# HDembinski/zenflow

Hardware: AMD Instinct MI355X
Metric: log_prob samples/sec (+ NLL match) 4D 16-knot 4-layer flow, batch 2^20 (higher is better)
Workload: dtype fp32 (f16x2 split MFMA, fp32 accumulate)

## Files before the change

### zenflow_amd/csrc/zf_flow.hip

```cpp
#include "zf_flow_dev.h"

#include <cmath>
#include <cstdlib>
#include <cstring>
#include <vector>

namespace zf {
namespace {

constexpr int kWaves = 4;
constexpr int kBlockRows = kWaves * kTile;

template <int T>
__device__ __forceinline__ floatx16 mfma_tile(const floatx4* __restrict__ p,
                                              const floatx4* __restrict__ pnext, floatx4 (&cur)[4],
                                              const floatx16 (&hb)[T]) {
  floatx16 acc = floatx16{0};
#pragma unroll
  for (int t = 0; t < T; ++t) {
    floatx4 nxt[4];
    const bool more = (t + 1 < T);
    const floatx4* src = more ? p + (t + 1) * 256 : pnext;
    const bool have = more || (pnext != nullptr);
    if (have) {
// ... 192 lines not shown

  flow_epilogue<kWaves>(F, xs, s, hh, lane, wave, rot, D, row, valid, ld, lp_out, block_partial, 1, 0,
                        y_out, ld_out, s_part);
}

__global__ __launch_bounds__(256) void latent_sample_kernel(int latent, float param, unsigned long long seed,
                                                            float* __restrict__ z, long long n, int D) {
  const long long i = (long long)blockIdx.x * 256 + threadIdx.x;
  if (i >= n) return;
  const long long row = i / D;
  const int d = (int)(i - row * D);
  z[i] = latent_draw(latent, param, seed, row, d);
}

constexpr int kReduceThreads = 1024;
__global__ __launch_bounds__(kReduceThreads) void reduce_partials(const double* __restrict__ part, long long n,
                                                                  double* __restrict__ out) {
  __shared__ double sm[kReduceThreads];
  const int t = threadIdx.x;
  double acc = 0.0;
  long long i = t;
  for (; i + 7 * kReduceThreads < n; i += 8 * kReduceThreads) {
    double v[8];
#pragma unroll
    for (int j = 0; j < 8; ++j) v[j] = part[i + j * kReduceThreads];
#pragma unroll
    for (int j = 0; j < 8; ++j) acc += v[j];
  }
  for (; i < n; i += kReduceThreads) acc += part[i];
  sm[t] = acc;
// ... 349 lines not shown
  if (e == hipSuccess && layered) {
    rcd = zf::layered_create(desc, nat, need, &h->lay);
    if (rcd) {
      zf_flow_destroy(h);
      return rcd;
    }
  }
  if (e == hipSuccess && use_x3) e = hipMalloc(&h->d_x3, x3s.size() * sizeof(uint16_t));
  if (e == hipSuccess && use_x3)
    e = hipMemcpy(h->d_x3, x3s.data(), x3s.size() * sizeof(uint16_t), hipMemcpyHostToDevice);
  if (e == hipSuccess) e = hipMalloc(&h->d_desc, sizeof(zf::DevFlow));
  if (e == hipSuccess) e = hipMalloc(&h->d_blob, h->packed.size() * sizeof(float) + 1024);
  if (e == hipSuccess) e = hipMemcpy(h->d_desc, &h->host, sizeof(zf::DevFlow), hipMemcpyHostToDevice);
  if (e == hipSuccess)
    e = hipMemcpy(h->d_blob, h->packed.data(), h->packed.size() * sizeof(float), hipMemcpyHostToDevice);
  if (e != hipSuccess) {
    rcd = zf::hip_status(e, "zf_flow_create");
    zf_flow_destroy(h);
    return rcd;
  }
  *handle = h;
  return ZF_OK;
}

int zf_flow_destroy(zf_flow_t* h) {
  if (!h) return ZF_OK;
  if (h->d_desc) (void)hipFree(h->d_desc);
  if (h->d_blob) (void)hipFree(h->d_blob);
  if (h->d_x3) (void)hipFree(h->d_x3);
  if (h->d_res_state) (void)hipFree(h->d_res_state);
// ... 43 lines not shown
    a.oact = h->x3_oact;
    a.aset = h->x3_aset;
    a.par_bytes = h->host.x3_par_bytes;
    a.seed = seed;
    a.gen = gen;
    a.stream = (hipStream_t)stream;
    a.latent = h->host.latent;
    a.sb_affine = true;
    for (int i = op_begin; i < op_end; ++i) {
      if (h->desc.ops[i].kind != ZF_OP_SHIFT_BOUNDS) continue;
      for (int j = 0; j < h->host.D; ++j) {
        const int mode = (int)h->packed[(size_t)h->host.ops[i].sb + 8 * j];
        if (mode != ZF_SB_NONE && mode != ZF_SB_BOTH) a.sb_affine = false;
      }
    }
    if (h->x3_res_mode != 0 && (h->x3_res_mode == 1 || N >= kX3ResidentAutoRows) &&
        x3_resident_fits(h->desc, a, INV, h->ncu)) {
      const long long need = ((long long)(N + kTile - 1) / kTile) * kTile * (h->host.D + 1);
      if (need > h->res_floats) {
        hipStreamCaptureStatus cs = hipStreamCaptureStatusNone;
        if (hipStreamIsCapturing(a.stream, &cs) == hipSuccess && cs == hipStreamCaptureStatusNone) {
          if (h->d_res_state) (void)hipFree(h->d_res_state);
          h->d_res_state = nullptr;
          h->res_floats = 0;
          ZF_TRY_HIP(hipMalloc(&h->d_res_state, (size_t)need * sizeof(float)));
          h->res_floats = need;
        }
      }
      if (need <= h->res_floats) a.res_state = h->d_res_state;
    }
// ... 143 lines not shown
```

### zenflow_amd/csrc/zf_flow_dev.h

```cpp
#pragma once
#include "zf_act.h"
#include "zf_internal.h"
#include "zf_random.h"
#include "zf_spline.h"

#include <cstdint>
#include <vector>

namespace zf {

typedef float floatx16 __attribute__((ext_vector_type(16)));
typedef float floatx4 __attribute__((ext_vector_type(4)));

constexpr int kTile = 32;
constexpr int kMaxOps = 64;

struct DevOp {
  int kind, shift, K, S;
  int n_hidden, dt, dc, DC;
  int KS0, T_last, nslot_mask, act;
  long long w[17];
  long long b[17];
  long long bn;
  long long sb;
// ... 6 lines not shown
  float x3_rb[16][2];
  int x3_par_pieces;
  long long x3_nbase[2], x3_nbn[2];
  int x3_npieces[2], x3_npar[2];
};

struct DevFlow {
  int D, C, latent, n_ops;
  int HP, nslot, per_wave, x3_ok;
  int small_floats;
  int x3_par_bytes;
  int kreal;
  int _pad;
  float lat_c0, lat_c1, lat_c2, lat_c3;
  DevOp ops[kMaxOps];
};

__device__ __forceinline__ void wave_lds_sync() {
  __builtin_amdgcn_fence(__ATOMIC_SEQ_CST, "wavefront");
  __builtin_amdgcn_wave_barrier();
}

__device__ __forceinline__ float swish(float v) {
  return v * __builtin_amdgcn_rcpf(1.0f + __builtin_amdgcn_exp2f(-v * 1.44269504f));
}

__device__ __forceinline__ float rcp_refined(float x) {
  float r = __builtin_amdgcn_rcpf(x);
  return __builtin_fmaf(__builtin_fmaf(-x, r, 1.0f), r, r);
}
// ... 28 lines not shown
  floatx16 a;
#pragma unroll
  for (int r = 0; r < 16; ++r) a[r] = b[r >> 2][r & 3];
  return a;
}

__device__ __forceinline__ int pmod(int a, int m) {
  int r = a % m;
  return r < 0 ? r + m : r;
}

__device__ __forceinline__ int wrap(int a, int m) { return a >= m ? a - m : a; }

struct KnotConsts {
  float c, norm, rnorm;
  __device__ __forceinline__ explicit KnotConsts(int K) {
    const double c64 = 1e-5 / (1.0 - (double)K * 1e-5);
    c = (float)c64;
    norm = (float)(1.0 + c64 * (double)K);
    rnorm = rcp_refined(norm);
  }
};

__device__ __forceinline__ void load_state(float* xs, const float* __restrict__ xin, long long row,
                                           bool valid, int D, int s, int hh, const DevFlow* __restrict__ F,
                                           unsigned long long seed, int gen) {
  for (int d = hh; d < D; d += 2) {
    float v = 0.f;
    if (valid) v = gen ? latent_draw(F->latent, F->lat_c3, seed, row, d) : xin[row * D + d];
    xs[d * 32 + s] = v;
// ... 158 lines not shown
      if (lane == 0) s_part[wave] = v;
      __syncthreads();
      if (threadIdx.x == 0) {
        double acc = 0.0;
        for (int w = 0; w < NW; ++w) acc += s_part[w];
        const long long b0 = slot >= 0 ? slot : (long long)blockIdx.x * pstride;
        block_partial[b0] = acc;
        for (int k = 1; k < pstride; ++k)
          if (b0 + k < nparts) block_partial[b0 + k] = 0.0;
      }
    }
  }
  flow_out_rows(xs, s, hh, rot, D, row, valid, ld, y_out, ld_out);
}

struct X3Launch {
  const DevFlow* desc;
  const float* blob;
  const void* x3;
  const float *x, *c;
  float* y;
  const float* ld_in;
  float *ld_out, *lp;
  double* part;
  long long nparts;
  int op_begin, op_end;
  long long N;
  unsigned long long seed;
  int gen;
  int K, D, C, T;
  int NT;
  bool oact;
  int aset;
  int par_bytes;
  float* res_state = nullptr;
  int res_blocks = 0, res_slots = 0, res_span = 0;
  bool sb_affine = false;
  int latent = 0;
  bool res_frame = false;
  hipStream_t stream;
};
int launch_flow_x3(const X3Launch& a, bool inverse);
int x3_resident_mode();
bool x3_resident_fits(const zf_flow_desc& desc, X3Launch& a, bool inverse, int ncu);
bool x3_eligible(const zf_flow_desc& desc, int HP, int* K);
struct LayeredFlow;
int layered_create(const zf_flow_desc& desc, const float* natural, int64_t n, LayeredFlow** out);
void layered_destroy(LayeredFlow* L);
int layered_run(LayeredFlow* L, const DevFlow& F, const float* packed, bool inverse, int op_begin, int op_end,
                const float* x, const float* c, float* y, const float* ld_in, float* ld_out, float* lp, double* part,
                long long N, hipStream_t st, unsigned long long seed, int gen);
int x3_last_tiles(int K);
// ... 10 lines not shown
```

### zenflow_amd/csrc/zf_flow_x3.hip

```cpp
#include "zf_flow_x3_kernel.h"

#include <cmath>
#include <cstdint>
#include <cstdlib>
#include <cstring>
#include <vector>

namespace zf {

int launch_x3_k8(const X3Launch& a, bool inverse);
int launch_x3_k16(const X3Launch& a, bool inverse);
int launch_x3_k32(const X3Launch& a, bool inverse);
int launch_x3_k64(const X3Launch& a, bool inverse);

namespace {

uint16_t bf16_rne(float f) {
  uint32_t u;
  std::memcpy(&u, &f, 4);
  if ((u & 0x7fffffffu) > 0x7f800000u) return (uint16_t)((u >> 16) | 0x40);
  u += 0x7fffu + ((u >> 16) & 1u);
  return (uint16_t)(u >> 16);
}

// ... 47 lines not shown
    if (desc.ops[i].n_hidden != 2) return false;
    if (i >= a.op_begin && i < a.op_end) in_range = true;
  }
  if (!in_range) return false;
  const int TL = dt == 1 ? x3_last_tiles_one(a.K) : x3_last_tiles(a.K);
  const long long span = 4ll * (2 * 4 * 2 * 1024) + 4ll * (2 * TL * 2 * 1024);
  const long long nslots = (a.N + 127) / 128;
  const long long slots = (nslots + ncu - 1) / ncu;
  if (slots > (1 << 20)) return false;
  if (x3_res_lds_bytes((size_t)span, a.par_bytes, a.D + a.C, 4 * slots, false) > 160 * 1024) return false;
  if (a.K != 16 || dt != 2) return false;
#ifndef ZF_X3R_FRAME
#define ZF_X3R_FRAME 1
#endif
  a.res_frame = ZF_X3R_FRAME && a.D == 4 && a.C == 0 && a.sb_affine && a.latent == ZF_LATENT_NORMAL &&
                a.ld_in == nullptr;
  for (int i = a.op_begin, run = 0; i < a.op_end && a.res_frame; ++i) {
    const int kind = desc.ops[i].kind;
    run = kind == ZF_OP_NSC ? 0 : run + (kind == ZF_OP_SHIFT_BOUNDS ? 1 : 0);
    if (run > 1) a.res_frame = false;
  }
  if (x3_res_lds_bytes((size_t)span, a.par_bytes, a.D + a.C, 4 * slots, true) > 160 * 1024) a.res_frame = false;
  a.res_blocks = ncu;
  a.res_slots = (int)slots;
  a.res_span = (int)span;
  return true;
}

int x3_padded_knots(int K) {
  if (K < 2) return 0;
  if (K <= 8) return 8;
  if (K <= 16) return 16;
  if (K <= 32) return 32;
// ... 220 lines not shown
```

### zenflow_amd/csrc/zf_flow_x3_k16_res.hip

```cpp
#include "zf_flow_x3_kernel.h"

namespace zf {

int launch_x3r_k16(const X3Launch& a, bool inverse) { return launch_x3r<16, false>(a, inverse); }

}
```

### zenflow_amd/csrc/zf_flow_x3_kernel.h

```cpp
#pragma once
#include "zf_flow_dev.h"

#include <cmath>
#include <cstdint>
#include <cstdlib>
#include <cstring>
#include <utility>
#include <vector>

namespace zf {
namespace {

typedef float floatx2 __attribute__((ext_vector_type(2)));
typedef __bf16 bf16x2 __attribute__((ext_vector_type(2)));
typedef __bf16 bf16x8 __attribute__((ext_vector_type(8)));
typedef _Float16 halfx2 __attribute__((ext_vector_type(2)));
typedef _Float16 halfx8 __attribute__((ext_vector_type(8)));

template <int NT>
struct XT;
template <>
struct XT<3> {
  using E = bf16x8;
  static constexpr int kProd = 6;
// ... 7 lines not shown
constexpr int kWideSched = 3;

#ifndef ZF_X3_WAVES
#define ZF_X3_WAVES 4
#endif
constexpr int kX3Waves = ZF_X3_WAVES;
static_assert(kX3Waves % 4 == 0, "whole 128-row NLL partial slots per block");

#ifndef ZF_X3_ABL
#define ZF_X3_ABL 0
#endif
#ifdef ZF_X3_TRACE
constexpr int kX3TraceSlots = 16;
__device__ unsigned long long* x3_trace_buf;
#define X3T_NOW() __builtin_amdgcn_s_memtime()
#endif
template <int NT>
constexpr int group_bytes(int NOUT) { return 2 * NOUT * NT * 1024; }


template <int S>
__device__ __forceinline__ void split8(const floatx16& v, bf16x8& bh, bf16x8& bm, bf16x8& bl) {
#pragma unroll
  for (int i = 0; i < 4; ++i) {
    const floatx2 x = {v[8 * S + 2 * i], v[8 * S + 2 * i + 1]};
    const bf16x2 h = __builtin_convertvector(x, bf16x2);
    const floatx2 r = x - __builtin_convertvector(h, floatx2);
    const bf16x2 m = __builtin_convertvector(r, bf16x2);
    const floatx2 r2 = r - __builtin_convertvector(m, floatx2);
    const bf16x2 l = __builtin_convertvector(r2, bf16x2);
// ... 897 lines not shown
  }
}

template <int NT, int T, int NOUT, bool SW, bool OACT, int Q = 0>
__device__ __forceinline__ void x3_layer(const char* __restrict__ x3, X3Pipe& p, floatx16 (&hb)[T],
                                         floatx16 (&acc)[NOUT], int lane, const float* bias_last, int hh,
                                         float isc, float us, int act) {
  if constexpr (Q + 1 < T) {
    x3_step<NT, T, NOUT, Q, SW, OACT>(x3, p, hb, acc, lane, nullptr, hh, isc, us, act);
    x3_layer<NT, T, NOUT, SW, OACT, Q + 1>(x3, p, hb, acc, lane, bias_last, hh, isc, us, act);
  } else {
    x3_step<NT, T, NOUT, Q, SW, OACT>(x3, p, hb, acc, lane, bias_last, hh, isc, us, act);
  }
}

template <int T, bool OACT>
__device__ __forceinline__ void x3_layer0(const X3Sc& c, const float* par, const float* xs, int rot, int D,
                                          int s, int hh, int lane, floatx16 (&hb)[T], int swish_tiles,
                                          float* umax = nullptr) {
  const int dt = c.dt, dc = c.dc, DC = c.DC, KS0 = c.KS0;
  const int DCp = 2 * KS0;
  const float* bn = par;
  const float* w0b = par + c.w0_rel;
  const float* b0 = par + c.b_rel;
#pragma unroll
  for (int o = 0; o < T; ++o) hb[o] = bias_acc(b0 + o * 32, hh);
  for (int ks = 0; ks < KS0; ++ks) {
    const int k = 2 * ks + hh;
    float v = 0.f;
    if (k < dc) v = xs[wrap(dt + k + rot, D) * 32 + s];
    else if (k < DC) v = xs[(D + k - dc) * 32 + s];
    const float u = (v - bn[k]) * bn[DCp + k] + bn[2 * DCp + k];
    if (umax != nullptr) *umax = fmaxf(*umax, fabsf(u));
    const float* w0 = w0b + ks * 64 + lane;
#pragma unroll
    for (int o = 0; o < T; ++o) hb[o] = __builtin_amdgcn_mfma_f32_32x32x2f32(w0[o * KS0 * 64], u, hb[o], 0, 0, 0);
  }
#pragma unroll
  for (int o = 0; o < T; ++o)
    if (o < swish_tiles) {
      if constexpr (OACT) {
        x3_act_tile<3, true>(hb[o], 1.f, c.act);
      } else {
#pragma unroll
        for (int r = 0; r < 16; ++r) hb[o][r] = swish(hb[o][r]);
      }
    }
}

__device__ __forceinline__ float x3_squareplus(float x) {
  return 0.5f * (x + __builtin_amdgcn_sqrtf(__builtin_fmaf(x, x, 4.0f)));
}

__device__ __forceinline__ float x3_squareplus2(float x) {
  return x + __builtin_amdgcn_sqrtf(__builtin_fmaf(x, x, 4.0f));
}

__device__ __forceinline__ void x3_forward_eval(float x, const RqsBin& b, float& y, float& ld) {
  const float rw = rcp_refined(b.w);
  const float sk = b.h * rw;
  const float zr = (x - b.xk) * rw;
  const float z = (zr != zr) ? zr : fminf(fmaxf(zr, kEps), kOneMinusEps);
  const float az = 1.0f - z;
  const float num = b.h * z * (sk * z + b.dk * az);
  const float den = sk + (b.dkp1 + b.dk - 2.0f * sk) * z * az;
  const float rd = rcp_refined(den + kEps);
  const float yv = b.yk + num * rd;
  y = b.oob ? x : yv;
  const float num2 = z * (b.dkp1 * z + 2.0f * sk * az) + b.dk * (az * az);
  const float sq = (sk + kEps) * rd;
  const float l = __logf((num2 + kEps) * (sq * sq));
  ld = b.oob ? 0.0f : l;
}

__device__ __forceinline__ float x3_sqrt_cr(float a) {
  const float y = __builtin_amdgcn_rsqf(a);
  const float sq = a * y;
  const float r = __builtin_fmaf(__builtin_fmaf(-sq, sq, a), 0.5f * y, sq);
  return a == __builtin_huge_valf() ? a : r;
}
template <bool CR>
__device__ __forceinline__ float x3_squareplus2_t(float x) {
  const float a = __builtin_fmaf(x, x, 4.0f);
  return x + (CR ? x3_sqrt_cr(a) : __builtin_amdgcn_sqrtf(a));
}
// ... 24 lines not shown
    for (int i = 0; i <= H; ++i) S2[i] = c ? S[H + i] : S[i];
    x3_bsel<FWD, H, H>(v, X2, Y2, W2, H2, S2, out);
  }
}

template <int K>
struct KnotLit {
  static constexpr double c64 = 1e-5 / (1.0 - (double)K * 1e-5);
  static constexpr float c = (float)c64;
  static constexpr float norm = (float)(1.0 + c64 * (double)K);
  static constexpr float rnorm = (float)(1.0 / (double)norm);
  static constexpr float bc = c * rnorm;
};

template <bool FWD, int K, bool CR, bool KLIT, int NPV>
__device__ __forceinline__ RqsBin x3_bin(float v, const float (&P)[NPV], const KnotConsts& kc) {
  float ws[K], hs[K];
#pragma unroll
  for (int j = 0; j < K; ++j) {
    ws[j] = x3_squareplus2_t<CR>(P[j]);
    hs[j] = x3_squareplus2_t<CR>(P[K + j]);
  }
  float X[K + 1], Y[K + 1];
  X[0] = 0.f;
  Y[0] = 0.f;
  X[1] = ws[0];
  Y[1] = hs[0];
#pragma unroll
  for (int j = 1; j < K; ++j) {
    X[j + 1] = X[j] + ws[j];
    Y[j + 1] = Y[j] + hs[j];
  }
  const float rn = KLIT ? KnotLit<K>::rnorm : kc.rnorm;
  const float bc = KLIT ? KnotLit<K>::bc : kc.c * kc.rnorm;
  const float ax = rcp_refined(X[K]) * rn, ay = rcp_refined(Y[K]) * rn;
#pragma unroll
  for (int j = 1; j <= K; ++j) {
    const float jb = KLIT ? (float)j * KnotLit<K>::bc : (float)j * bc;
    X[j] = __builtin_fmaf(X[j], ax, jb);
    Y[j] = __builtin_fmaf(Y[j], ay, jb);
  }
  float S[K + 1];
  S[0] = 0.f;
  S[K] = 0.f;
#pragma unroll
  for (int j = 1; j < K; ++j) S[j] = P[2 * K + j - 1];
  float o[6];
  x3_bsel<FWD, K, K + 1>(v, X, Y, ws, hs, S, o);
  RqsBin b;
// ... 20 lines not shown
  unsigned long long t_last;
};
#define X3T(k)                                   \
  {                                              \
    const unsigned long long t_ = X3T_NOW();     \
    tr.tacc[k] += t_ - tr.t_last;                \
    tr.t_last = t_;                              \
  }
#elif defined(ZF_X3_MARK)
struct X3Tr {};
#define X3T(k) asm volatile(";ZFMARK " #k)
#else
struct X3Tr {};
#define X3T(k)
#endif
#ifdef ZF_X3_MARK
#define X3M(k) asm volatile(";ZFMARK " #k)
#else
#define X3M(k)
#endif

template <int NT, int K, int T, bool PAIRS, bool ONE, bool INV, bool OACT, int ASET, bool RES>
__device__ __forceinline__ void x3_nsc(const DevOp& op, const X3Sc& opc, const char* __restrict__ x3, X3Pipe& pipe,
                                       const float* par, float* xs, int rot, int D, int s, int hh, int lane,
                                       float& ld, X3Tr& tr) {
  constexpr int TL = ONE ? (3 * K - 1 + 31) / 32 : (3 * K - 1 + 15) / 16;
  constexpr int NPV = ONE ? 32 * TL : 16 * TL;
  const int nh = opc.nh, act = opc.act, dt = opc.dt, kw_last = opc.kw_last;
  const KnotConsts kc(opc.kreal);
  const bool padlast = opc.kreal == K - 1;
#ifdef ZF_X3_MARK
  const bool klit = true;
#else
  const bool klit = opc.kreal == K;
#endif
  const long long b_rel = opc.b_rel + T * 32, blast_rel = opc.blast_rel;
  floatx16 hb[T];
  constexpr bool kLastSW = !PAIRS;
  constexpr bool kPipe = T == 4 && !PAIRS;
#ifndef ZF_X3_EARLY
#define ZF_X3_EARLY 1
#endif
  constexpr bool kEarly = ZF_X3_EARLY && NT == 2 && !OACT && kPipe;
  static_assert(!RES || kEarly, "the resident form runs the early-scale slot schedule only");
#ifndef ZF_X3_PRESP
#define ZF_X3_PRESP 1
#endif
  constexpr int kPreSP = (!ZF_X3_PRESP || !kEarly) ? 0 : !ONE ? K / 8 : (K == 16 ? 1 : 0);
  float umax = 0.f;
  x3_layer0<T, OACT>(opc, par, xs, rot, D, s, hh, lane, hb, NT == 2 ? 0 : (!OACT && (nh > 1 || kLastSW)) ? 1 : T,
                     kEarly ? &umax : nullptr);
  float eU = 0.f, eisc = 1.f, eus = 1.f, eius = 1.f;
  halfx8 ecs[2];
  if constexpr (kEarly) {
    const X3Halves uq = x3_halves(umax);
    umax = fmaxf(uq.lo, uq.hi);
    eU = __builtin_fmaf(op.x3_rb[0][0], umax, op.x3_rb[0][1]);
    x3_scale_from(eU, nh > 1 ? opc.kw1 : kw_last, eisc, eus, eius);
    x3_act_tile<NT, false>(hb[0], eisc, act);
    split8h<0>(hb[0], ecs[0], ecs[1]);
  }
#ifndef ZF_X3_SEEDSCALED
#define ZF_X3_SEEDSCALED 0
#endif
  constexpr bool kSeedScaled = NT == 2 && (ZF_X3_SEEDSCALED || !kPipe);
#ifndef ZF_X3_WIDE_PIPE
#define ZF_X3_WIDE_PIPE 1
#endif
#ifndef ZF_X3_PAIRS_PIPE
#define ZF_X3_PAIRS_PIPE 1
#endif
  constexpr bool kPipeH = kPipe || (ZF_X3_PAIRS_PIPE && (T == 4 || ZF_X3_WIDE_PIPE) && NT == 2 && !OACT);
#ifndef ZF_X3_ACTIN
#define ZF_X3_ACTIN 1
#endif
  constexpr bool kActIn = ZF_X3_ACTIN && NT == 2 && ASET == 2 && kPipeH;
  constexpr bool kSeedScaledH = NT == 2 && (ZF_X3_SEEDSCALED || !kPipeH);
#if ZF_X3_ABL != 4
  if constexpr (T == 4) __builtin_amdgcn_s_setprio(2);
#endif
  X3T(1);
  if constexpr (kEarly) {
    float eM = eU;
    for (int l = 1; l < nh; ++l) {
      const float nU = __builtin_fmaf(op.x3_rb[l][0], eM, op.x3_rb[l][1]);
      float nisc, nus, nius;
      x3_scale_from(nU, l + 1 < nh ? op.x3_kw[l + 1] : kw_last, nisc, nus, nius);
      floatx16 acc[T];
#pragma unroll
      for (int o = 0; o < T; ++o) acc[o] = floatx16{0};
      float mx;
      x3_layer_early<T, T, true, 0, 0, RES>(x3, pipe, hb, acc, lane, par + b_rel + (l - 1) * (T * 32), hh, ecs, eisc, eus,
                                 nisc, mx);
#pragma unroll
      for (int o = 0; o < T; ++o) hb[o] = acc[o];
      eU = nU; eisc = nisc; eus = nus; eius = nius;
      const X3Halves mq = x3_halves(mx);
      eM = fmaxf(mq.lo, mq.hi);
    }
  } else
  for (int l = 1; l < nh; ++l) {
    floatx16 acc[T];
    float isc = 1.f, us = 1.f, ius = 1.f;
    if constexpr (NT == 2) {
      x3_act_scale<T, OACT>(hb, l == 1 ? opc.kw1 : op.x3_kw[l], isc, us, ius, act);
#pragma unroll
      for (int o = 0; o < (OACT && !kActIn ? T : 1); ++o) x3_act_tile<NT, OACT, ASET>(hb[o], isc, act);
    }
    const float* bl_l = par + b_rel + (l - 1) * (T * 32);
#pragma unroll
    for (int o = 0; o < T; ++o)
      acc[o] = NT == 3 ? bias_acc(bl_l + o * 32, hh)
                       : (kSeedScaledH ? bias_acc(bl_l + o * 32, hh) * ius : floatx16{0});
    const float* bh = (NT == 2 && !kSeedScaledH) ? bl_l : nullptr;
    if constexpr (kPipeH) {
      typename XT<NT>::E cs[NT];
      splitk<NT, 0>(hb[0], cs);
      halfx8 fs1[2];
      x3_layer_pipe<NT, T, T, NT == 2 && !kSeedScaledH, OACT, 0, kActIn ? ASET : 0>(x3, pipe, hb, acc, lane, bh, hh,
                                                                                 cs, isc, us,
// ... 9 lines not shown
#pragma unroll
    for (int o = 0; o < T; ++o) {
      if (o < nsw) {
        if constexpr (OACT) {
          hb[o] = acc[o];
          x3_act_tile<3, true>(hb[o], 1.f, act);
        } else {
#pragma unroll
          for (int r = 0; r < 16; ++r) hb[o][r] = swish(acc[o][r]);
        }
      } else {
        hb[o] = acc[o];
      }
    }
  }
  X3T(2);
  float ldn = 0.f;
  const int npair = PAIRS ? (dt + 1) / 2 : 1;
  float lisc = 1.f, lus = 1.f, lius = 1.f;
  if constexpr (kEarly) {
    lisc = eisc; lus = eus; lius = eius;
  } else if constexpr (NT == 2) {
    x3_act_scale<T, OACT>(hb, kw_last, lisc, lus, lius, act);
#pragma unroll
    for (int o = 0; o < T; ++o)
      if (o == 0 || !kLastSW || (OACT && !(kActIn && kPipe))) x3_act_tile<NT, OACT, ASET>(hb[o], lisc, act);
  }
#ifndef ZF_X3_PRESPLIT
#define ZF_X3_PRESPLIT 1
#endif
  constexpr bool kPre = ZF_X3_PRESPLIT && PAIRS && T == 4 && NT == 2 && !OACT;
  halfx8 sp[kPre ? T : 1][2][2];
  if constexpr (kPre) {
#pragma unroll
    for (int q = 0; q < T; ++q) {
      split8h<0>(hb[q], sp[q][0][0], sp[q][0][1]);
      split8h<1>(hb[q], sp[q][1][0], sp[q][1][1]);
    }
  }
  for (int pr = 0; pr < npair; ++pr) {
    const float* bl = par + blast_rel + pr * TL * 32;
    floatx16 pa[TL];
    constexpr bool kSeed = PAIRS && NT == 3;
#pragma unroll
    for (int o = 0; o < TL; ++o)
      pa[o] = kSeed ? bias_acc(bl + o * 32, hh) : (kSeedScaled ? bias_acc(bl + o * 32, hh) * lius : floatx16{0});
    X3T(3);
    if constexpr (kEarly) {
      float mx;
      x3_layer_early<T, TL, false, kPreSP, 0, RES>(x3, pipe, hb, pa, lane, bl, hh, ecs, lisc, lus, 0.f, mx);
    } else if constexpr (kPre) {
      x3_layer_pre<T, TL>(x3, pipe, sp, pa, lane);
    } else if constexpr (kPipe) {
      typename XT<NT>::E cs[NT];
      splitk<NT, 0>(hb[0], cs);
      halfx8 fs1[2];
      x3_layer_pipe<NT, T, TL, !kSeedScaled, OACT, 0, kActIn ? ASET : 0>(x3, pipe, hb, pa, lane, bl, hh, cs, lisc,
                                                                         lus, act, fs1);
    } else {
      x3_layer<NT, T, TL, kLastSW, OACT>(x3, pipe, hb, pa, lane, (kSeed || kSeedScaled) ? nullptr : bl, hh,
                                         lisc, lus, act);
    }
    if constexpr (kSeedScaled) {
#pragma unroll
      for (int o = 0; o < TL; ++o) pa[o] *= lus;
    }
    if constexpr (T == 4) __builtin_amdgcn_s_setprio(0);
    X3T(4);
    constexpr bool kSplitWH = ONE && K == 16;
    float P[NPV];
#pragma unroll
    for (int o = 0; o < TL; ++o)
#pragma unroll
      for (int r = 0; r < 16; ++r) {
        if constexpr (kSplitWH) {
          if (o == 0) P[r] = pa[0][r];
          else
            P[2 * K + r] = x3_halves(pa[1][r]).lo;
        } else if constexpr (ONE) {
          const X3Halves q = x3_halves(pa[o][r]);
          P[32 * o + r] = q.lo;
          P[32 * o + 16 + r] = q.hi;
        } else {
// ... 10 lines not shown
    }
#endif
    const int d = 2 * pr + hh;
    const bool dact = d < dt;
    float ldv = 0.f;
    {
      float* xp = xs + wrap((dact ? d : 0) + rot, D) * 32 + s;
      const float xv = *xp;
#ifndef ZF_X3_BSEARCH
#define ZF_X3_BSEARCH 0
#endif
      RqsBin bin;
      bool binned = false;
      if constexpr (ZF_X3_BSEARCH && !kSplitWH && !kPreSP && (K == 8 || K == 16 || K == 32 || K == 64)) {
        if (klit) {
          bin = x3_bin<!INV, K, OACT, true>(xv, P, kc);
          binned = true;
        }
      }
      if (!binned) {
        float w[K], hg[K];
        const float bc = kc.c * kc.rnorm;
        if constexpr (kSplitWH) {
          float sw = 0.f;
#pragma unroll
          for (int j = 0; j < K; ++j) {
            w[j] = kPreSP ? P[j] : x3_squareplus2_t<OACT>(P[j]);
            sw = sw + w[j];
          }
          const float a = rcp_refined(sw) * kc.rnorm;
#pragma unroll
          for (int j = 0; j < K; ++j) {
            const X3Halves q = x3_halves(__builtin_fmaf(w[j], a, bc));
            w[j] = q.lo;
            hg[j] = q.hi;
          }
        } else {
          float sx = 0.f, sy = 0.f;
#pragma unroll
          for (int j = 0; j < K; ++j) {
            w[j] = kPreSP ? P[j] : x3_squareplus2_t<OACT>(P[j]);
            hg[j] = kPreSP ? P[K + j] : x3_squareplus2_t<OACT>(P[K + j]);
            sx = sx + w[j];
            sy = sy + hg[j];
          }
          const float ax = rcp_refined(sx) * kc.rnorm, ay = rcp_refined(sy) * kc.rnorm;
#pragma unroll
          for (int j = 0; j < K; ++j) {
            w[j] = __builtin_fmaf(w[j], ax, bc);
            hg[j] = __builtin_fmaf(hg[j], ay, bc);
          }
        }
        X3M(12);
        float sl[K - 1];
#pragma unroll
        for (int j = 0; j < K - 1; ++j) sl[j] = P[2 * K + j];
#ifndef ZF_X3_EXECBIN
#define ZF_X3_EXECBIN 1
#endif
        const auto spf = [](float v) { return v == 0.f ? 1.f : x3_squareplus_t<OACT>(v); };
        if constexpr (ZF_X3_EXECBIN && K % 8 == 0) bin = rqs_bin_exec<!INV, K>(xv, w, hg, sl, spf, padlast);
// ... 6 lines not shown
        x3_forward_eval(xv, bin, yv, l);
        ldv = dact ? l : 0.f;
      } else {
        yv = rqs_inverse_eval(xv, bin);
      }
      if (dact) *xp = yv;
    }
    wave_lds_sync();
    if (!INV) {
      const X3Halves q = x3_halves(ldv);
      ldn = ldn + q.lo;
      if (2 * pr + 1 < dt) ldn = ldn + q.hi;
    }
  }
  if (!INV) ld = ld + ldn;
  X3T(5);
}

constexpr int kX3ResWaves = 12;

inline size_t x3_res_lds_bytes(size_t span, int par_bytes, int DS, long long tiles_per_block, bool frame) {
  return span + (size_t)par_bytes + (size_t)kX3ResWaves * 2 * (DS + 1) * 32 * 4 + (size_t)tiles_per_block * 8 +
         (frame ? 128 : 0);
}

__device__ __forceinline__ void x3r_fetch(const float* __restrict__ st, float* buf, int D, int DS, int lane) {
#pragma nounroll
  for (int j = 0; j < D; j += 2)
    if (j + (lane >> 5) < D)
      __builtin_amdgcn_global_load_lds((const void*)(st + j * 32 + lane),
                                       (__attribute__((address_space(3))) void*)(buf + j * 32), 4, 0, 0);
// ... 125 lines not shown
  float* xs0 = reinterpret_cast<float*>(par_lds + PB) + wave * (2 * SB);
  double* s_part = reinterpret_cast<double*>(reinterpret_cast<float*>(par_lds + PB) + NW * 2 * SB);
  const long long slot0 = (long long)blockIdx.x * slots_per_block;
  const long long tile0 = slot0 * 4;
  const long long left = (N + kTile - 1) / kTile - tile0;
  const int nt = left <= 0 ? 0 : (left < 4ll * slots_per_block ? (int)left : 4 * slots_per_block);
  for (int i = threadIdx.x; i < 4 * slots_per_block; i += NW * 64) s_part[i] = 0.0;

  X3Pipe pipe;
  pipe.nxt = nullptr;
  pipe.wave = wave;
  pipe.par_src = nullptr;
  pipe.par_dst = nullptr;
  pipe.par_pieces = 0;
  X3Tr tr = {};
  const int nq = op_end - op_begin;
  int rot0 = 0;
  bool first = true;
  floatx4* sbk = reinterpret_cast<floatx4*>(s_part + 4 * slots_per_block);
  for (int q = 0; q < nq;) {
    int nsc = -1, seg_end = nq;
    for (int r = q; r < nq; ++r)
      if (F->ops[INV ? (op_end - 1 - r) : (op_begin + r)].kind == ZF_OP_NSC) {
        if (nsc < 0) {
          nsc = r;
        } else {
          seg_end = nsc + 1;
          break;
        }
      }
// ... 10 lines not shown
        } else if (kind == ZF_OP_SHIFT_BOUNDS) {
          if (r < nsc) {
            fr_sba = oi;
            fr_rota = rot;
          } else {
            fr_sbb = oi;
            fr_rotb = rot;
          }
        } else {
          fr_nsc = oi;
          fr_rotn = rot;
        }
      }
      fr_pack = X3rPass::pack(fr_rota, fr_rotb, fr_rotn, rot, fr_sba >= 0, fr_sbb >= 0, fr_nsc);
    }
    __syncthreads();
    if (nsc >= 0 && nt > 0) {
      const DevOp& fo = F->ops[INV ? (op_end - 1 - nsc) : (op_begin + nsc)];
      const int pieces = (T * (fo.n_hidden - 1) * group_bytes<NT>(T) + T * group_bytes<NT>(fo.x3_tlast)) >> 10;
      x3_dma(x3 + fo.x3, lds, pieces, wave, lane, NW);
      x3_dma(reinterpret_cast<const char*>(blob + fo.bn), par_lds, fo.x3_par_pieces, wave, lane, NW);
    }
    if constexpr (FR) {
      int lh = lane;
      asm volatile("" : "+v"(lh));
      if (wave == 0 && lh < 8) {
        const int oi = lh < 4 ? fr_sba : fr_sbb;
        if (oi >= 0) sbk[lh] = x3r_sb_consts<INV>(blob + F->ops[oi].sb, lh & 3);
      }
    }
    asm volatile("s_waitcnt vmcnt(0)" ::: "memory");
    __syncthreads();

    int cur = 0;
    if (!first && wave < nt) x3r_fetch(state + (tile0 + wave) * ST, xs0, D, DS, lane);
    float lat_c0 = 0.f, lat_c1 = 1.f;
    if (FR && last && lp_out != nullptr) {
      lat_c0 = F->lat_c0;
      lat_c1 = F->lat_c1;
    }
    for (int t = wave; t < nt; t += NW) {
      float* xs = xs0 + cur * SB;
      const long long tile = tile0 + t;
      const long long nleft = N - tile * kTile;
      const int nrows = nleft < kTile ? (int)nleft : kTile;
      int ln = lane;
      asm volatile("" : "+v"(ln));
      {
        const int s1 = ln & 31, h1 = ln >> 5;
        const long long row1 = tile * kTile + s1;
        const bool valid1 = FR ? s1 < nrows : row1 < N;
        if (first) {
          if constexpr (FR) {
            const float lat_c3 = F->lat_c3;
            const float* xt = xin + tile * (kTile * 4);
#pragma unroll
            for (int d = h1; d < 4; d += 2) {
              float v = 0.f;
              if (valid1) v = (INV && gen) ? latent_draw(ZF_LATENT_NORMAL, lat_c3, seed, row1, d) : xt[s1 * 4 + d];
              xs[d * 32 + s1] = v;
            }
          } else {
            load_state(xs, xin, row1, valid1, D, s1, h1, F, seed, INV ? gen : 0);
          }
        } else if (t == wave) {
          asm volatile("s_waitcnt vmcnt(0)" ::: "memory");
        }
#pragma nounroll
        for (int j = h1; j < C; j += 2) xs[(D + j) * 32 + s1] = valid1 ? cin[row1 * C + j] : 0.f;
      }
      wave_lds_sync();
      float ld;
      if (first) {
        const long long row1 = tile * kTile + (ln & 31);
        ld = (!FR && ld_in != nullptr && row1 < N) ? ld_in[row1] : 0.f;
      } else {
        ld = xs[DS * 32 + (ln & 31)];
        if (t + NW < nt) x3r_fetch(state + (tile + NW) * ST, xs0 + (cur ^ 1) * SB, D, DS, ln);
      }
      int rot = rot0;
      if constexpr (FR) {
        int fp = fr_pack;
        asm volatile("" : "+s"(fp));
        if (X3rPass::has_sb_before(fp)) x3r_shift_bounds<INV>(sbk, xs, s, hh, X3rPass::rot_sb_before(fp), ld);
        {
          const DevOp& op = F->ops[X3rPass::nsc(fp)];
          const X3Sc opc = x3_scalars<INV>(op);
          int zoff = 0;
          asm volatile("" : "+s"(zoff));
          pipe.cur = lds + zoff;
          pipe.g = 0;
          x3_nsc<NT, K, T, false, ONE, INV, false, 0, true>(
              op, opc, x3, pipe, reinterpret_cast<const float*>(par_lds + zoff), xs, X3rPass::rot_nsc(fp), 4, s, hh, lane, ld,
              tr);
        }
        asm volatile("" : "+s"(fp));
        if (X3rPass::has_sb_after(fp)) x3r_shift_bounds<INV>(sbk + 4, xs, s, hh, X3rPass::rot_sb_after(fp), ld);
        rot = X3rPass::rot_end(fp);
      } else {
        for (int r = q; r < seg_end; ++r) {
          const DevOp& op = F->ops[INV ? (op_end - 1 - r) : (op_begin + r)];
          const X3Sc opc = x3_scalars<INV>(op);
          if (opc.kind == ZF_OP_ROLL) {
            rot = pmod(INV ? rot + opc.shift : rot - opc.shift, D);
          } else if (opc.kind == ZF_OP_SHIFT_BOUNDS) {
            shift_bounds_op<INV>(blob + opc.sb, xs, s, hh, rot, D, ld);
          } else {
            int zoff = 0;
            asm volatile("" : "+s"(zoff));
            pipe.cur = lds + zoff;
            pipe.g = 0;
            x3_nsc<NT, K, T, false, ONE, INV, false, 0, true>(
                op, opc, x3, pipe, reinterpret_cast<const float*>(par_lds + zoff), xs, rot, D, s, hh, lane, ld, tr);
          }
        }
      }
      asm volatile("s_waitcnt vmcnt(0)" ::: "memory");
      asm volatile("" : "+v"(ln));
      const int s2 = ln & 31, h2 = ln >> 5;
      const long long row = tile * kTile + s2;
      const bool valid = FR ? s2 < nrows : row < N;
      if (!last) {
        float* st = state + tile * ST;
        if constexpr (FR) {
#pragma unroll
          for (int d = h2; d < 4; d += 2) st[d * 32 + s2] = xs[d * 32 + s2];
        } else {
#pragma nounroll
          for (int d = h2; d < D; d += 2) st[d * 32 + s2] = xs[d * 32 + s2];
        }
        if (h2 == 0) st[D * 32 + s2] = ld;
      } else if constexpr (FR) {
        if (lp_out != nullptr) {
          const double v = x3r_lp_rows(lat_c0, lat_c1, xs, s2, h2, rot, valid, ld, lp_out + tile * kTile,
                                       block_partial != nullptr);
          if (block_partial != nullptr && ln == 0) s_part[t] = v;
        }
        if (y_out != nullptr && valid) {
          float* yt = y_out + tile * (kTile * 4);
#pragma unroll
          for (int j = h2; j < 4; j += 2) yt[s2 * 4 + j] = xs[((j + rot) & 3) * 32 + s2];
        }
        if (ld_out != nullptr && valid && h2 == 0) (ld_out + tile * kTile)[s2] = ld;
      } else {
        if (lp_out != nullptr) {
          const double v = flow_lp_rows(F, xs, s2, h2, rot, D, row, valid, ld, lp_out, block_partial != nullptr);
          if (block_partial != nullptr && ln == 0) s_part[t] = v;
        }
        flow_out_rows(xs, s2, h2, rot, D, row, valid, ld, y_out, ld_out);
      }
      wave_lds_sync();
      cur ^= 1;
    }
    for (int r = q; r < seg_end; ++r) {
      const DevOp& op = F->ops[INV ? (op_end - 1 - r) : (op_begin + r)];
      if (op.kind == ZF_OP_ROLL) rot0 = pmod(INV ? rot0 + op.shift : rot0 - op.shift, D);
    }
    q = seg_end;
    first = false;
  }
  __syncthreads();
  if (lp_out != nullptr && block_partial != nullptr) {
    const int ns = (nt + 3) / 4;
    for (int i = threadIdx.x; i < ns; i += NW * 64) {
      double acc = 0.0;
      for (int w = 0; w < 4; ++w) acc += s_part[4 * i + w];
// ... 189 lines not shown
```

Baseline: 1.461 billion.

## Specialize resident frame NSC path with literal layout and precomputed knot constants

```diff
diff --git a/zenflow_amd/csrc/zf_flow.hip b/zenflow_amd/csrc/zf_flow.hip
--- a/zenflow_amd/csrc/zf_flow.hip
+++ b/zenflow_amd/csrc/zf_flow.hip
@@ -230,6 +230,19 @@
 }
 
 constexpr int kReduceThreads = 1024;
+__global__ __launch_bounds__(64) void knot_consts_kernel(DevFlow* F) {
+  if (threadIdx.x != 0 || blockIdx.x != 0) return;
+  for (int i = 0; i < F->n_ops; ++i) {
+    const DevOp& op = F->ops[i];
+    if (op.kind != ZF_OP_NSC) continue;
+    const KnotConsts kc(op.K);
+    F->kc[i][0] = kc.c;
+    F->kc[i][1] = kc.norm;
+    F->kc[i][2] = kc.rnorm;
+    F->kc[i][3] = 0.f;
+  }
+}
+
 __global__ __launch_bounds__(kReduceThreads) void reduce_partials(const double* __restrict__ part, long long n,
                                                                   double* __restrict__ out) {
   __shared__ double sm[kReduceThreads];
@@ -609,6 +622,11 @@
   if (e == hipSuccess) e = hipMemcpy(h->d_desc, &h->host, sizeof(zf::DevFlow), hipMemcpyHostToDevice);
   if (e == hipSuccess)
     e = hipMemcpy(h->d_blob, h->packed.data(), h->packed.size() * sizeof(float), hipMemcpyHostToDevice);
+  if (e == hipSuccess) {
+    hipLaunchKernelGGL(zf::knot_consts_kernel, dim3(1), dim3(64), 0, (hipStream_t) nullptr, h->d_desc);
+    e = hipGetLastError();
+  }
+  if (e == hipSuccess) e = hipMemcpy(&h->host, h->d_desc, sizeof(zf::DevFlow), hipMemcpyDeviceToHost);
   if (e != hipSuccess) {
     rcd = zf::hip_status(e, "zf_flow_create");
     zf_flow_destroy(h);
@@ -682,6 +700,14 @@
         if (mode != ZF_SB_NONE && mode != ZF_SB_BOTH) a.sb_affine = false;
       }
     }
+    a.par_lit = true;
+    for (int i = op_begin; i < op_end; ++i) {
+      const DevOp& d = h->host.ops[i];
+      if (d.kind != ZF_OP_NSC) continue;
+      if (d.w[0] - d.bn != X3Lit::kW0 || d.b[0] - d.bn != X3Lit::kB0 || d.b[1] - d.b[0] != 128 ||
+          d.x3_blast - d.bn != X3Lit::blast(a.K))
+        a.par_lit = false;
+    }
     if (h->x3_res_mode != 0 && (h->x3_res_mode == 1 || N >= kX3ResidentAutoRows) &&
         x3_resident_fits(h->desc, a, INV, h->ncu)) {
       const long long need = ((long long)(N + kTile - 1) / kTile) * kTile * (h->host.D + 1);
diff --git a/zenflow_amd/csrc/zf_flow_dev.h b/zenflow_amd/csrc/zf_flow_dev.h
--- a/zenflow_amd/csrc/zf_flow_dev.h
+++ b/zenflow_amd/csrc/zf_flow_dev.h
@@ -44,6 +44,7 @@
   int _pad;
   float lat_c0, lat_c1, lat_c2, lat_c3;
   DevOp ops[kMaxOps];
+  float kc[kMaxOps][4];
 };
 
 __device__ __forceinline__ void wave_lds_sync() {
@@ -102,6 +103,7 @@
 
 struct KnotConsts {
   float c, norm, rnorm;
+  __device__ __forceinline__ explicit KnotConsts(const float (&k)[4]) : c(k[0]), norm(k[1]), rnorm(k[2]) {}
   __device__ __forceinline__ explicit KnotConsts(int K) {
     const double c64 = 1e-5 / (1.0 - (double)K * 1e-5);
     c = (float)c64;
@@ -290,6 +292,15 @@
   flow_out_rows(xs, s, hh, rot, D, row, valid, ld, y_out, ld_out);
 }
 
+struct X3Lit {
+  static constexpr int kW0 = 8;
+  static constexpr int kB0 = kW0 + 4 * 64;
+  static constexpr int blast(int K) { return kB0 + 2 * 128 + (2 * (3 * K - 1) + 31) / 32 * 32; }
+  float bc, rnorm;
+  float rb[2][2];
+  int kw1, kw_last;
+};
+
 struct X3Launch {
   const DevFlow* desc;
   const float* blob;
@@ -312,6 +323,7 @@
   float* res_state = nullptr;
   int res_blocks = 0, res_slots = 0, res_span = 0;
   bool sb_affine = false;
+  bool par_lit = false;
   int latent = 0;
   bool res_frame = false;
   hipStream_t stream;
diff --git a/zenflow_amd/csrc/zf_flow_x3.hip b/zenflow_amd/csrc/zf_flow_x3.hip
--- a/zenflow_amd/csrc/zf_flow_x3.hip
+++ b/zenflow_amd/csrc/zf_flow_x3.hip
@@ -85,9 +85,10 @@
 #define ZF_X3R_FRAME 1
 #endif
   a.res_frame = ZF_X3R_FRAME && a.D == 4 && a.C == 0 && a.sb_affine && a.latent == ZF_LATENT_NORMAL &&
-                a.ld_in == nullptr;
+                a.ld_in == nullptr && a.par_lit;
   for (int i = a.op_begin, run = 0; i < a.op_end && a.res_frame; ++i) {
     const int kind = desc.ops[i].kind;
+    if (kind == ZF_OP_NSC && desc.ops[i].knots != a.K) a.res_frame = false;
     run = kind == ZF_OP_NSC ? 0 : run + (kind == ZF_OP_SHIFT_BOUNDS ? 1 : 0);
     if (run > 1) a.res_frame = false;
   }
diff --git a/zenflow_amd/csrc/zf_flow_x3_k16_res.hip b/zenflow_amd/csrc/zf_flow_x3_k16_res.hip
--- a/zenflow_amd/csrc/zf_flow_x3_k16_res.hip
+++ b/zenflow_amd/csrc/zf_flow_x3_k16_res.hip
@@ -5,3 +5,10 @@
 int launch_x3r_k16(const X3Launch& a, bool inverse) { return launch_x3r<16, false>(a, inverse); }
 
 }
+
+#ifdef ZF_X3_TRACE
+extern "C" int zf_x3r_trace_set_k16(void* buf, long long n) {
+  if (hipMemcpyToSymbol(HIP_SYMBOL(zf::x3r_trace_buf), &buf, sizeof(buf)) != hipSuccess) return 1;
+  return hipMemcpyToSymbol(HIP_SYMBOL(zf::x3r_trace_cap), &n, sizeof(n)) == hipSuccess ? 0 : 1;
+}
+#endif
diff --git a/zenflow_amd/csrc/zf_flow_x3_kernel.h b/zenflow_amd/csrc/zf_flow_x3_kernel.h
--- a/zenflow_amd/csrc/zf_flow_x3_kernel.h
+++ b/zenflow_amd/csrc/zf_flow_x3_kernel.h
@@ -45,6 +45,16 @@
 constexpr int kX3TraceSlots = 16;
 __device__ unsigned long long* x3_trace_buf;
 #define X3T_NOW() __builtin_amdgcn_s_memtime()
+constexpr int kX3rStamps = 16, kX3rTracePasses = 4;
+__device__ unsigned long long* x3r_trace_buf;
+__device__ long long x3r_trace_cap;
+#define X3R_STAMP(slot)                                                                       \
+  {                                                                                           \
+    const long long i_ = x3r_tix + (slot);                                                    \
+    if (x3r_tb != nullptr && lane == 0 && (slot) < kX3rStamps && i_ < x3r_cap) x3r_tb[i_] = X3T_NOW(); \
+  }
+#else
+#define X3R_STAMP(slot)
 #endif
 template <int NT>
 constexpr int group_bytes(int NOUT) { return 2 * NOUT * NT * 1024; }
@@ -972,15 +982,23 @@
   }
 }
 
-template <int T, bool OACT>
+template <int T, bool OACT, bool LIT = false>
 __device__ __forceinline__ void x3_layer0(const X3Sc& c, const float* par, const float* xs, int rot, int D,
                                           int s, int hh, int lane, floatx16 (&hb)[T], int swish_tiles,
                                           float* umax = nullptr) {
-  const int dt = c.dt, dc = c.dc, DC = c.DC, KS0 = c.KS0;
+  int dt, dc, DC, KS0;
+  long long w0_rel, b_rel;
+  if constexpr (LIT) {
+    dt = 2; dc = 2; DC = 2; KS0 = 1;
+    w0_rel = X3Lit::kW0; b_rel = X3Lit::kB0;
+  } else {
+    dt = c.dt; dc = c.dc; DC = c.DC; KS0 = c.KS0;
+    w0_rel = c.w0_rel; b_rel = c.b_rel;
+  }
   const int DCp = 2 * KS0;
   const float* bn = par;
-  const float* w0b = par + c.w0_rel;
-  const float* b0 = par + c.b_rel;
+  const float* w0b = par + w0_rel;
+  const float* b0 = par + b_rel;
 #pragma unroll
   for (int o = 0; o < T; ++o) hb[o] = bias_acc(b0 + o * 32, hh);
   for (int ks = 0; ks < KS0; ++ks) {
@@ -998,6 +1016,7 @@
   for (int o = 0; o < T; ++o)
     if (o < swish_tiles) {
       if constexpr (OACT) {
+        static_assert(!(OACT && LIT), "the literal body is swish only");
         x3_act_tile<3, true>(hb[o], 1.f, c.act);
       } else {
 #pragma unroll
@@ -1026,7 +1045,12 @@
   const float yv = b.yk + num * rd;
   y = b.oob ? x : yv;
   const float num2 = z * (b.dkp1 * z + 2.0f * sk * az) + b.dk * (az * az);
-  const float sq = (sk + kEps) * rd;
+  float ske;
+  {
+#pragma clang fp contract(off)
+    ske = sk + kEps;
+  }
+  const float sq = ske * rd;
   const float l = __logf((num2 + kEps) * (sq * sq));
   ld = b.oob ? 0.0f : l;
 }
@@ -1081,7 +1105,7 @@
 };
 
 template <bool FWD, int K, bool CR, bool KLIT, int NPV>
-__device__ __forceinline__ RqsBin x3_bin(float v, const float (&P)[NPV], const KnotConsts& kc) {
+__device__ __forceinline__ RqsBin x3_bin(float v, const float (&P)[NPV], float krn, float kbc) {
   float ws[K], hs[K];
 #pragma unroll
   for (int j = 0; j < K; ++j) {
@@ -1098,8 +1122,8 @@
     X[j + 1] = X[j] + ws[j];
     Y[j + 1] = Y[j] + hs[j];
   }
-  const float rn = KLIT ? KnotLit<K>::rnorm : kc.rnorm;
-  const float bc = KLIT ? KnotLit<K>::bc : kc.c * kc.rnorm;
+  const float rn = KLIT ? KnotLit<K>::rnorm : krn;
+  const float bc = KLIT ? KnotLit<K>::bc : kbc;
   const float ax = rcp_refined(X[K]) * rn, ay = rcp_refined(Y[K]) * rn;
 #pragma unroll
   for (int j = 1; j <= K; ++j) {
@@ -1150,27 +1174,64 @@
 struct X3Tr {};
 #define X3T(k)
 #endif
+#ifdef ZF_X3_TRACE
+#define X3TN(k) if constexpr (!RES) X3T(k)
+#else
+#define X3TN(k) X3T(k)
+#endif
 #ifdef ZF_X3_MARK
 #define X3M(k) asm volatile(";ZFMARK " #k)
 #else
 #define X3M(k)
 #endif
 
-template <int NT, int K, int T, bool PAIRS, bool ONE, bool INV, bool OACT, int ASET, bool RES>
+template <int NT, int K, int T, bool PAIRS, bool ONE, bool INV, bool OACT, int ASET, bool RES, bool LIT = false>
 __device__ __forceinline__ void x3_nsc(const DevOp& op, const X3Sc& opc, const char* __restrict__ x3, X3Pipe& pipe,
                                        const float* par, float* xs, int rot, int D, int s, int hh, int lane,
-                                       float& ld, X3Tr& tr) {
+                                       float& ld, X3Tr& tr, const X3Lit& lit = X3Lit{}) {
+  static_assert(!LIT || (RES && T == 4 && !PAIRS && !ONE && !OACT && NT == 2), "the frame's shape");
   constexpr int TL = ONE ? (3 * K - 1 + 31) / 32 : (3 * K - 1 + 15) / 16;
   constexpr int NPV = ONE ? 32 * TL : 16 * TL;
-  const int nh = opc.nh, act = opc.act, dt = opc.dt, kw_last = opc.kw_last;
-  const KnotConsts kc(opc.kreal);
-  const bool padlast = opc.kreal == K - 1;
+  int nh, act, dt, kw1, kw_last;
+  long long b0_rel, blast_rel;
+  float krn, kcc = 0.f, kbc_res = 0.f;
+  bool padlast, klit;
+  if constexpr (LIT) {
+    nh = 2; act = ZF_ACT_SWISH; dt = 2;
+    kw1 = lit.kw1; kw_last = lit.kw_last;
+    b0_rel = X3Lit::kB0; blast_rel = X3Lit::blast(K);
+    padlast = false; klit = true;
+    krn = lit.rnorm; kbc_res = lit.bc;
+  } else {
+    nh = opc.nh; act = opc.act; dt = opc.dt;
+    kw_last = opc.kw_last;
+    if constexpr (RES) {
+      krn = lit.rnorm; kbc_res = lit.bc;
+    } else {
+      const KnotConsts kc(opc.kreal);
+      krn = kc.rnorm; kcc = kc.c;
+    }
+    padlast = opc.kreal == K - 1;
+    klit = opc.kreal == K;
+    b0_rel = opc.b_rel; blast_rel = opc.blast_rel;
+    kw1 = opc.kw1;
+  }
+  const auto kbc = [&]() -> float {
+    if constexpr (RES) return kbc_res;
+    else return kcc * krn;
+  };
+  const auto rb = [&](int l, int j) -> float {
+    if constexpr (LIT) return lit.rb[l & 1][j];
+    else return op.x3_rb[l][j];
+  };
+  const auto kwl = [&](int l) -> int {
+    if constexpr (LIT) return l == 1 ? lit.kw1 : lit.kw_last;
+    else return op.x3_kw[l];
+  };
 #ifdef ZF_X3_MARK
-  const bool klit = true;
-#else
-  const bool klit = opc.kreal == K;
-#endif
-  const long long b_rel = opc.b_rel + T * 32, blast_rel = opc.blast_rel;
+  klit = true;
+#endif
+  const long long b_rel = b0_rel + T * 32;
   floatx16 hb[T];
   constexpr bool kLastSW = !PAIRS;
   constexpr bool kPipe = T == 4 && !PAIRS;
@@ -1184,15 +1245,15 @@
 #endif
   constexpr int kPreSP = (!ZF_X3_PRESP || !kEarly) ? 0 : !ONE ? K / 8 : (K == 16 ? 1 : 0);
   float umax = 0.f;
-  x3_layer0<T, OACT>(opc, par, xs, rot, D, s, hh, lane, hb, NT == 2 ? 0 : (!OACT && (nh > 1 || kLastSW)) ? 1 : T,
+  x3_layer0<T, OACT, LIT>(opc, par, xs, rot, D, s, hh, lane, hb, NT == 2 ? 0 : (!OACT && (nh > 1 || kLastSW)) ? 1 : T,
                      kEarly ? &umax : nullptr);
   float eU = 0.f, eisc = 1.f, eus = 1.f, eius = 1.f;
   halfx8 ecs[2];
   if constexpr (kEarly) {
     const X3Halves uq = x3_halves(umax);
     umax = fmaxf(uq.lo, uq.hi);
-    eU = __builtin_fmaf(op.x3_rb[0][0], umax, op.x3_rb[0][1]);
-    x3_scale_from(eU, nh > 1 ? opc.kw1 : kw_last, eisc, eus, eius);
+    eU = __builtin_fmaf(rb(0, 0), umax, rb(0, 1));
+    x3_scale_from(eU, nh > 1 ? kw1 : kw_last, eisc, eus, eius);
     x3_act_tile<NT, false>(hb[0], eisc, act);
     split8h<0>(hb[0], ecs[0], ecs[1]);
   }
@@ -1215,13 +1276,13 @@
 #if ZF_X3_ABL != 4
   if constexpr (T == 4) __builtin_amdgcn_s_setprio(2);
 #endif
-  X3T(1);
+  X3TN(1);
   if constexpr (kEarly) {
     float eM = eU;
     for (int l = 1; l < nh; ++l) {
-      const float nU = __builtin_fmaf(op.x3_rb[l][0], eM, op.x3_rb[l][1]);
+      const float nU = __builtin_fmaf(rb(l, 0), eM, rb(l, 1));
       float nisc, nus, nius;
-      x3_scale_from(nU, l + 1 < nh ? op.x3_kw[l + 1] : kw_last, nisc, nus, nius);
+      x3_scale_from(nU, l + 1 < nh ? kwl(l + 1) : kw_last, nisc, nus, nius);
       floatx16 acc[T];
 #pragma unroll
       for (int o = 0; o < T; ++o) acc[o] = floatx16{0};
@@ -1239,7 +1300,7 @@
     floatx16 acc[T];
     float isc = 1.f, us = 1.f, ius = 1.f;
     if constexpr (NT == 2) {
-      x3_act_scale<T, OACT>(hb, l == 1 ? opc.kw1 : op.x3_kw[l], isc, us, ius, act);
+      x3_act_scale<T, OACT>(hb, l == 1 ? kw1 : kwl(l), isc, us, ius, act);
 #pragma unroll
       for (int o = 0; o < (OACT && !kActIn ? T : 1); ++o) x3_act_tile<NT, OACT, ASET>(hb[o], isc, act);
     }
@@ -1279,7 +1340,7 @@
       }
     }
   }
-  X3T(2);
+  X3TN(2);
   float ldn = 0.f;
   const int npair = PAIRS ? (dt + 1) / 2 : 1;
   float lisc = 1.f, lus = 1.f, lius = 1.f;
@@ -1310,7 +1371,7 @@
 #pragma unroll
     for (int o = 0; o < TL; ++o)
       pa[o] = kSeed ? bias_acc(bl + o * 32, hh) : (kSeedScaled ? bias_acc(bl + o * 32, hh) * lius : floatx16{0});
-    X3T(3);
+    X3TN(3);
     if constexpr (kEarly) {
       float mx;
       x3_layer_early<T, TL, false, kPreSP, 0, RES>(x3, pipe, hb, pa, lane, bl, hh, ecs, lisc, lus, 0.f, mx);
@@ -1331,7 +1392,7 @@
       for (int o = 0; o < TL; ++o) pa[o] *= lus;
     }
     if constexpr (T == 4) __builtin_amdgcn_s_setprio(0);
-    X3T(4);
+    X3TN(4);
     constexpr bool kSplitWH = ONE && K == 16;
     float P[NPV];
 #pragma unroll
@@ -1372,13 +1433,13 @@
       bool binned = false;
       if constexpr (ZF_X3_BSEARCH && !kSplitWH && !kPreSP && (K == 8 || K == 16 || K == 32 || K == 64)) {
         if (klit) {
-          bin = x3_bin<!INV, K, OACT, true>(xv, P, kc);
+          bin = x3_bin<!INV, K, OACT, true>(xv, P, krn, kbc());
           binned = true;
         }
       }
       if (!binned) {
         float w[K], hg[K];
-        const float bc = kc.c * kc.rnorm;
+        const float bc = kbc();
         if constexpr (kSplitWH) {
           float sw = 0.f;
 #pragma unroll
@@ -1386,7 +1447,7 @@
             w[j] = kPreSP ? P[j] : x3_squareplus2_t<OACT>(P[j]);
             sw = sw + w[j];
           }
-          const float a = rcp_refined(sw) * kc.rnorm;
+          const float a = rcp_refined(sw) * krn;
 #pragma unroll
           for (int j = 0; j < K; ++j) {
             const X3Halves q = x3_halves(__builtin_fmaf(w[j], a, bc));
@@ -1402,7 +1463,7 @@
             sx = sx + w[j];
             sy = sy + hg[j];
           }
-          const float ax = rcp_refined(sx) * kc.rnorm, ay = rcp_refined(sy) * kc.rnorm;
+          const float ax = rcp_refined(sx) * krn, ay = rcp_refined(sy) * krn;
 #pragma unroll
           for (int j = 0; j < K; ++j) {
             w[j] = __builtin_fmaf(w[j], ax, bc);
@@ -1439,7 +1500,7 @@
     }
   }
   if (!INV) ld = ld + ldn;
-  X3T(5);
+  X3TN(5);
 }
 
 constexpr int kX3ResWaves = 12;
@@ -1595,6 +1656,11 @@
   pipe.par_dst = nullptr;
   pipe.par_pieces = 0;
   X3Tr tr = {};
+#ifdef ZF_X3_TRACE
+  unsigned long long* const x3r_tb = x3r_trace_buf;
+  const long long x3r_cap = x3r_trace_cap;
+  int x3r_pass = 0;
+#endif
   const int nq = op_end - op_begin;
   int rot0 = 0;
   bool first = true;
@@ -1635,14 +1701,36 @@
       }
       fr_pack = X3rPass::pack(fr_rota, fr_rotb, fr_rotn, rot, fr_sba >= 0, fr_sbb >= 0, fr_nsc);
     }
+#ifdef ZF_X3_TRACE
+    const long long x3r_tix = x3r_pass < kX3rTracePasses
+                                  ? (((long long)blockIdx.x * NW + wave) * kX3rTracePasses + x3r_pass) * kX3rStamps
+                                  : x3r_cap;
+    ++x3r_pass;
+#endif
+    X3R_STAMP(0);
     __syncthreads();
+    X3R_STAMP(1);
     if (nsc >= 0 && nt > 0) {
       const DevOp& fo = F->ops[INV ? (op_end - 1 - nsc) : (op_begin + nsc)];
       const int pieces = (T * (fo.n_hidden - 1) * group_bytes<NT>(T) + T * group_bytes<NT>(fo.x3_tlast)) >> 10;
       x3_dma(x3 + fo.x3, lds, pieces, wave, lane, NW);
       x3_dma(reinterpret_cast<const char*>(blob + fo.bn), par_lds, fo.x3_par_pieces, wave, lane, NW);
     }
+    X3R_STAMP(2);
+    X3Lit lit = {};
+    if (nsc >= 0) {
+      const KnotConsts kc(F->kc[INV ? (op_end - 1 - nsc) : (op_begin + nsc)]);
+      lit.bc = __int_as_float(__builtin_amdgcn_readfirstlane(__float_as_int(kc.c * kc.rnorm)));
+      lit.rnorm = __int_as_float(__builtin_amdgcn_readfirstlane(__float_as_int(kc.rnorm)));
+    }
     if constexpr (FR) {
+      if (nsc >= 0) {
+        const DevOp& fo = F->ops[INV ? (op_end - 1 - nsc) : (op_begin + nsc)];
+        lit.rb[0][0] = fo.x3_rb[0][0]; lit.rb[0][1] = fo.x3_rb[0][1];
+        lit.rb[1][0] = fo.x3_rb[1][0]; lit.rb[1][1] = fo.x3_rb[1][1];
+        lit.kw1 = fo.x3_kw[1];
+        lit.kw_last = fo.x3_kw[2];
+      }
       int lh = lane;
       asm volatile("" : "+v"(lh));
       if (wave == 0 && lh < 8) {
@@ -1652,6 +1740,7 @@
     }
     asm volatile("s_waitcnt vmcnt(0)" ::: "memory");
     __syncthreads();
+    X3R_STAMP(3);
 
     int cur = 0;
     if (!first && wave < nt) x3r_fetch(state + (tile0 + wave) * ST, xs0, D, DS, lane);
@@ -1676,7 +1765,8 @@
             const float lat_c3 = F->lat_c3;
             const float* xt = xin + tile * (kTile * 4);
 #pragma unroll
-            for (int d = h1; d < 4; d += 2) {
+            for (int e = 0; e < 2; ++e) {
+              const int d = h1 + 2 * e;
               float v = 0.f;
               if (valid1) v = (INV && gen) ? latent_draw(ZF_LATENT_NORMAL, lat_c3, seed, row1, d) : xt[s1 * 4 + d];
               xs[d * 32 + s1] = v;
@@ -1691,6 +1781,9 @@
         for (int j = h1; j < C; j += 2) xs[(D + j) * 32 + s1] = valid1 ? cin[row1 * C + j] : 0.f;
       }
       wave_lds_sync();
+#ifdef ZF_X3_TRACE
+      if (t == wave) X3R_STAMP(4);
+#endif
       float ld;
       if (first) {
         const long long row1 = tile * kTile + (ln & 31);
@@ -1706,14 +1799,14 @@
         if (X3rPass::has_sb_before(fp)) x3r_shift_bounds<INV>(sbk, xs, s, hh, X3rPass::rot_sb_before(fp), ld);
         {
           const DevOp& op = F->ops[X3rPass::nsc(fp)];
-          const X3Sc opc = x3_scalars<INV>(op);
+          const X3Sc opc = {};
           int zoff = 0;
           asm volatile("" : "+s"(zoff));
           pipe.cur = lds + zoff;
           pipe.g = 0;
-          x3_nsc<NT, K, T, false, ONE, INV, false, 0, true>(
-              op, opc, x3, pipe, reinterpret_cast<const float*>(par_lds + zoff), xs, X3rPass::rot_nsc(fp), 4, s, hh, lane, ld,
-              tr);
+          x3_nsc<NT, K, T, false, ONE, INV, false, 0, true, FR>(
+              op, opc, x3, pipe, reinterpret_cast<const float*>(par_lds + zoff), xs, X3rPass::rot_nsc(fp), 4, s, hh,
+              lane, ld, tr, lit);
         }
         asm volatile("" : "+s"(fp));
         if (X3rPass::has_sb_after(fp)) x3r_shift_bounds<INV>(sbk + 4, xs, s, hh, X3rPass::rot_sb_after(fp), ld);
@@ -1732,7 +1825,7 @@
             pipe.cur = lds + zoff;
             pipe.g = 0;
             x3_nsc<NT, K, T, false, ONE, INV, false, 0, true>(
-                op, opc, x3, pipe, reinterpret_cast<const float*>(par_lds + zoff), xs, rot, D, s, hh, lane, ld, tr);
+                op, opc, x3, pipe, reinterpret_cast<const float*>(par_lds + zoff), xs, rot, D, s, hh, lane, ld, tr, lit);
           }
         }
       }
@@ -1745,7 +1838,7 @@
         float* st = state + tile * ST;
         if constexpr (FR) {
 #pragma unroll
-          for (int d = h2; d < 4; d += 2) st[d * 32 + s2] = xs[d * 32 + s2];
+          for (int e = 0; e < 2; ++e) st[(h2 + 2 * e) * 32 + s2] = xs[(h2 + 2 * e) * 32 + s2];
         } else {
 #pragma nounroll
           for (int d = h2; d < D; d += 2) st[d * 32 + s2] = xs[d * 32 + s2];
@@ -1760,7 +1853,7 @@
         if (y_out != nullptr && valid) {
           float* yt = y_out + tile * (kTile * 4);
 #pragma unroll
-          for (int j = h2; j < 4; j += 2) yt[s2 * 4 + j] = xs[((j + rot) & 3) * 32 + s2];
+          for (int e = 0; e < 2; ++e) yt[s2 * 4 + h2 + 2 * e] = xs[((h2 + 2 * e + rot) & 3) * 32 + s2];
         }
         if (ld_out != nullptr && valid && h2 == 0) (ld_out + tile * kTile)[s2] = ld;
       } else {
@@ -1771,6 +1864,9 @@
         flow_out_rows(xs, s2, h2, rot, D, row, valid, ld, y_out, ld_out);
       }
       wave_lds_sync();
+#ifdef ZF_X3_TRACE
+      X3R_STAMP(5 + (t - wave) / NW);
+#endif
       cur ^= 1;
     }
     for (int r = q; r < seg_end; ++r) {
```

New measurement: 1.503 billion (median of 6 runs). 1.03x the previous value.
